# hartikainen/mujoco_mpc

Measured on AMD Instinct MI355X. Metric: candidate rollouts/s (horizon x samples), higher is better.
Workload: dtype f64

## Files before the change

mujoco_mpc_amd/csrc/constraint.h:

```cpp
#pragma once
DEV double impedance(const double *solimp_in, double pos, double margin) {
  double si0 = d_clip(solimp_in[0], 0.0001, 0.9999), si1 = d_clip(solimp_in[1], 0.0001, 0.9999);
  double si2 = fmax(0.0, solimp_in[2]), si3 = d_clip(solimp_in[3], 0.0001, 0.9999), si4 = fmax(1.0, solimp_in[4]);
  if (si0 == si1 || si2 <= D_MINVAL) return 0.5 * (si0 + si1);
  double x = d_div(pos - margin, si2);
  if (x < 0) x = -x;
  if (x >= 1) return si1;
  if (x == 0) return si0;
  double y;
  if (si4 == 1) y = x;
  else {
    int low = x <= si3;
    double m = low ? si3 : 1 - si3, u = low ? x : 1 - x;
    double a = d_div(1.0, d_pow_small(m, si4 - 1));
    double w = a * d_pow_small(u, si4);
    y = low ? w : 1 - w;
  }
  return si0 + y * (si1 - si0);
}

DEV double ball_angle(double *axis, const double *quat) {
  axis[0] = quat[1]; axis[1] = quat[2]; axis[2] = quat[3];
  double s = sqrt(axis[0] * axis[0] + axis[1] * axis[1] + axis[2] * axis[2]);
  if (s < D_MINVAL) { axis[0] = 1; axis[1] = 0; axis[2] = 0; } else { axis[0] /= s; axis[1] /= s; axis[2] /= s; }
// ... 180 lines not shown
        for (int w = MI(tendon_adr)[t2]; w < MI(tendon_adr)[t2] + MI(tendon_num)[t2]; w++) { int qa = MI(wrap_qposadr)[w]; dif += MD(wrap_prm)[w] * (c.qpos[qa] - MDH(qpos0)[qa]); }
        double deriv = ep[1] + dif * (2 * ep[2] + dif * (3 * ep[3] + dif * 4 * ep[4]));
        for (int w = MI(tendon_adr)[t2]; w < MI(tendon_adr)[t2] + MI(tendon_num)[t2]; w++) c.efc_J[r0 * nvp + MI(wrap_dofadr)[w]] -= deriv * MD(wrap_prm)[w];
      }
    } else {
      int b1 = et[1], b2 = et[2];
      const int weld = et[0] == 1;
      double p1[3], p2[3], quat[4], quat1[4];
      d_mulmatvec3(p1, c.xmat + 9 * b1, weld ? ep + 3 : ep); d_mulmatvec3(p2, c.xmat + 9 * b2, weld ? ep : ep + 3);
      for (int q = 0; q < 3; q++) { p1[q] += c.xpos[3 * b1 + q]; p2[q] += c.xpos[3 * b2 + q]; }
      if (weld) {
        d_mulquat(quat, c.xquat + 4 * b1, ep + 6);
        quat1[0] = c.xquat[4 * b2]; for (int q = 1; q < 4; q++) quat1[q] = -c.xquat[4 * b2 + q];
      }
      for (int d = 0; d < nv; d++) {
        unsigned long long bit = 1ull << d;
        int in1 = (MDM()[b1] & bit) != 0, in2 = (MDM()[b2] & bit) != 0;
        if (!in1 && !in2) continue;
        const double *cd = c.cdof + 6 * d;
        double jp[3] = {0, 0, 0}, off[3], t[3];
        if (in1) { d_sub3(off, p1, c.subtree_com + 3 * MIH(body_rootid)[b1]); d_cross(t, cd, off); for (int q = 0; q < 3; q++) jp[q] += cd[3 + q] + t[q]; }
        if (in2) { d_sub3(off, p2, c.subtree_com + 3 * MIH(body_rootid)[b2]); d_cross(t, cd, off); for (int q = 0; q < 3; q++) jp[q] -= cd[3 + q] + t[q]; }
        for (int q = 0; q < 3; q++) c.efc_J[(r0 + q) * nvp + d] = jp[q];
        if (weld) {
          double ax[4] = {0, 0, 0, 0}, tq[4], q3[4];
          if (in1) for (int q = 0; q < 3; q++) ax[1 + q] = cd[q];
          if (in2) for (int q = 0; q < 3; q++) ax[1 + q] -= cd[q];
          d_mulquat(tq, quat1, ax); d_mulquat(q3, tq, quat);
          for (int q = 0; q < 3; q++) c.efc_J[(r0 + 3 + q) * nvp + d] = ep[10] * (0.5 * q3[1 + q]);
        }
      }
    }
  }
  PFOR(rr, ntf_end - neq_end) {
    int r = neq_end + rr, t = MI(tfric_id)[c.efc_id[r]];
    for (int w = MI(tendon_adr)[t]; w < MI(tendon_adr)[t] + MI(tendon_num)[t]; w++) c.efc_J[r * nvp + MI(wrap_dofadr)[w]] = MD(wrap_prm)[w];
  }
  PFOR(rr, nball_end - ntf_end) {
    int r = ntf_end + rr, j = c.efc_id[r], da = MIH(jnt_dofadr)[j];
    double axis[3];
    ball_angle(axis, c.qpos + MIH(jnt_qposadr)[j]);
    for (int k = 0; k < 3; k++) c.efc_J[r * nvp + da + k] = -axis[k];
  }
  PFOR(rr, ntl_end - ntl0) {
    int r = ntl0 + rr, t = c.efc_id[r];
    double sg = c.efc_floss[r];
    for (int w = MI(tendon_adr)[t]; w < MI(tendon_adr)[t] + MI(tendon_num)[t]; w++) c.efc_J[r * nvp + MI(wrap_dofadr)[w]] = sg * MD(wrap_prm)[w];
    c.efc_floss[r] = 0;
  }
  SYNC();
  *nsingle_out = nlim_end; *n_nc_out = ntl_end;
}

DEV void make_contact_rows(Ctx &c, int n_nc) {
  const DevModel &M = *c.M;
  int nv = M.nv, nvp = M.nvp;
  int nefc = n_nc;
  for (int base = 0; base < c.ncon; base += NLANE) {
    int ci = base + LANE, dim = 0;
    if (ci < c.ncon) {
      dim = c.con_i[ci * CONI_STRIDE];
      if (dim > 1 && M.cone != 1) dim = 2 * (dim - 1);
    }
    int tot, off = wave_excl_scan(dim, &tot);
    if (nefc + tot > M.nefcmax) { c.warning |= WARN_CNSTRFULL; c.ncon = base; break; }
    if (ci < c.ncon) {
      int r0 = nefc + off;
      c.con_i[ci * CONI_STRIDE + 3] = r0;
      int g1 = c.con_i[ci * CONI_STRIDE + 1], g2 = c.con_i[ci * CONI_STRIDE + 2];
      int b1 = MI(geom_bodyid)[g1], b2 = MI(geom_bodyid)[g2];
      double tran = MDH(body_invweight0)[2 * b1] + MDH(body_invweight0)[2 * b2];
      double rot = MDH(body_invweight0)[2 * b1 + 1] + MDH(body_invweight0)[2 * b2 + 1];
      const double *cc = c.contact + ci * c.M->con_stride;
      int cdim = c.con_i[ci * CONI_STRIDE];
      int pyr = (cdim > 1 && M.cone != 1);
      for (int k = 0; k < dim; k++) {
        c.efc_type[r0 + k] = cdim == 1 ? CNSTR_CONTACT_FRICTIONLESS : (pyr ? CNSTR_CONTACT_PYRAMIDAL : CNSTR_CONTACT_ELLIPTIC);
        c.efc_id[r0 + k] = EFC_CON_ID(ci, cdim, r0);
        c.efc_floss[r0 + k] = 0; c.efc_pos[r0 + k] = cc[CON_DIST]; c.efc_margin[r0 + k] = cc[CON_INCLUDEMARGIN];
        if (pyr) { double mu = cc[CON_FRICTION + k / 2]; c.efc_diag[r0 + k] = tran + mu * mu * (k < 4 ? tran : rot); }
        else c.efc_diag[r0 + k] = k < 3 ? tran : rot;
      }
    }
    nefc += tot;
  }
  c.nefc = nefc;
  int crossflag = 0;
  PFOR(ci, c.ncon) {
    unsigned long long m1 = MPM()[MI(geom_bodyid)[c.con_i[ci * CONI_STRIDE + 1]]];
    unsigned long long m2 = MPM()[MI(geom_bodyid)[c.con_i[ci * CONI_STRIDE + 2]]];
    unsigned long long u = m1 | m2;
    if (u != m1 && u != m2) crossflag = 1;
  }
  c.cross = wave_or_i(crossflag) | M.limit_cross;
  SYNC();
  PFOR(e, (nefc - n_nc) * nvp) c.efc_J[n_nc * nvp + e] = 0;
  SYNC();
  int je_ci = LANE / nv, je_d = LANE - je_ci * nv;
  const int je_sq = NLANE / nv, je_sr = NLANE - je_sq * nv;
  for (int e = LANE; e < c.ncon * nv; e += NLANE, je_ci += je_sq, je_d += je_sr) {
    if (je_d >= nv) { je_d -= nv; je_ci++; }
    const int ci = je_ci, d = je_d;
    const int *cin = c.con_i + ci * CONI_STRIDE;
    int dim = cin[0], r0 = cin[3];
    int pyr = (dim > 1 && M.cone != 1);
    int b1 = MI(geom_bodyid)[cin[1]], b2 = MI(geom_bodyid)[cin[2]];
    unsigned long long bit = 1ull << d;
    int in1 = (MDM()[b1] & bit) != 0, in2 = (MDM()[b2] & bit) != 0;
    if (!in1 && !in2) continue;
    const double *cc = c.contact + ci * c.M->con_stride;
    const double *cd = c.cdof + 6 * d;
    double jp[3] = {0, 0, 0}, jr[3] = {0, 0, 0};
    if (in2) {
      double off[3], t[3];
      d_sub3(off, cc + CON_POS, c.subtree_com + 3 * MIH(body_rootid)[b2]);
      d_cross(t, cd, off);
      jp[0] += cd[3] + t[0]; jp[1] += cd[4] + t[1]; jp[2] += cd[5] + t[2];
      jr[0] += cd[0]; jr[1] += cd[1]; jr[2] += cd[2];
    }
    if (in1) {
      double off[3], t[3];
      d_sub3(off, cc + CON_POS, c.subtree_com + 3 * MIH(body_rootid)[b1]);
      d_cross(t, cd, off);
      jp[0] -= cd[3] + t[0]; jp[1] -= cd[4] + t[1]; jp[2] -= cd[5] + t[2];
      jr[0] -= cd[0]; jr[1] -= cd[1]; jr[2] -= cd[2];
    }
    if (pyr) {
      double jn = cc[CON_FRAME] * jp[0] + cc[CON_FRAME + 1] * jp[1] + cc[CON_FRAME + 2] * jp[2];
      for (int k = 1; k < dim; k++) {
        const double *ax = cc + CON_FRAME + 3 * (k % 3);
        const double *jj = k < 3 ? jp : jr;
        double jk = ax[0] * jj[0] + ax[1] * jj[1] + ax[2] * jj[2], mu = cc[CON_FRICTION + k - 1];
        c.efc_J[(r0 + 2 * (k - 1)) * nvp + d] = jn + mu * jk;
        c.efc_J[(r0 + 2 * (k - 1) + 1) * nvp + d] = jn - mu * jk;
      }
    } else {
      for (int k = 0; k < dim; k++) {
        const double *ax = cc + CON_FRAME + 3 * (k % 3);
        const double *jj = k < 3 ? jp : jr;
        c.efc_J[(r0 + k) * nvp + d] = ax[0] * jj[0] + ax[1] * jj[1] + ax[2] * jj[2];
      }
    }
  }
  SYNC();
}

DEV void make_impedance(Ctx &c, int r0, int r1, int with_contacts) {
  const DevModel &M = *c.M;
  int nv = M.nv, nvp = M.nvp;
  PFOR(rr, r1 - r0) {
    int r = r0 + rr;
    int type = c.efc_type[r], id = c.efc_id[r];
    double vel = 0;
    if (type == CNSTR_FRICTION_DOF) vel = c.qvel[id];
    else
// ... 78 lines not shown
```

mujoco_mpc_amd/csrc/core.h:

```cpp
#pragma once
#include "dmath.h"
#include "model.h"
#include "linalg.h"
#include "philox.h"

#ifdef MJPC_EMU
static thread_local double *g_emu_lds = nullptr;
static thread_local int g_emu_r = 0;
typedef const KParams *KP;
DEV const KParams *kp_generic(KP k) { return k; }
DEV double *lds_base() { return g_emu_lds; }
DEV int cand_index() { return g_emu_r; }
DEV int uniform_i(int v) { return v; }
#else
extern __shared__ __align__(16) double g_lds[];
typedef const __attribute__((address_space(4))) KParams *KP;
DEV const KParams *kp_generic(KP k) {
  unsigned long long v = (unsigned long long)k;
  unsigned lo = __builtin_amdgcn_readfirstlane((unsigned)v), hi = __builtin_amdgcn_readfirstlane((unsigned)(v >> 32));
  KP u = (KP)(((unsigned long long)hi << 32) | lo);
  return (const KParams *)u;
}
DEV double *lds_base() { return g_lds; }
DEV int cand_index() { return (int)blockIdx.x; }
// ... 233 lines not shown
    for (int k = 0; k < 9; k++) { c.xmat[k] = (k % 4 == 0) ? 1.0 : 0.0; c.ximat[k] = c.xmat[k]; }
    for (int k = 0; k < 6; k++) { c.cvel[k] = 0; c.cfrc[k] = 0; c.cacc[k] = (k >= 3) ? -M.gravity[k - 3] : 0.0; }
    for (int k = 0; k < MISC_INTS; k++) c.misc[k] = 0;
#if defined(MJPC_PROFILE) && !defined(MJPC_EMU)
    for (int q = 0; q < NPROF; q++) c.prof[q] = 0;
    c.prof[NPROF] = (long long)__builtin_amdgcn_s_memtime();
#endif
  }
  c.time = K->time;
  ctx_close(c);
}

template <int NVT>
DEV_NOINLINE void ph_head(KP Kc, int t, int last) {
  Ctx c; ctx_open(c, Kc);
  const KParams *K = c.K;
  const DevModel &M = *c.M;
  Rows R = out_rows(K);
  int nu = M.nu;
  if (!last) {
    PFOR(k, nu) {
      double a = spline_sample(c.knot_times, c.knot_values, K->P, nu, K->interp, c.time, k);
      a = d_clip(a, MD(actuator_ctrlrange)[2 * k], MD(actuator_ctrlrange)[2 * k + 1]);
      c.ctrl[k] = a; R.actions[t * nu + k] = a;
    }
    SYNC();
    if (bad_values(c.qpos, M.nq)) c.warning |= WARN_BADQPOS;
    if (bad_values(c.qvel, M.nv)) c.warning |= WARN_BADQVEL;
    if (c.warning) { if (LANE == 0) c.misc[MISC_BAD_STATE] = 1; ctx_close(c); return; }
    if (K->xfrc_std > 0) {
      double rate = exp(-M.timestep / K->xfrc_rate), scale = K->xfrc_std * sqrt(1 - rate * rate);
      unsigned gi = (unsigned)(K->offset + cand_index());
      int n6 = 6 * M.nbody;
      PFOR(i, n6) c.xfrc[i] = rate * c.xfrc[i] + scale * philox_normal(K->seed, K->stream ^ XFRC_STREAM, gi, (unsigned)(t * n6 + i));
    }
  }
  PROF(c, 0);
  kinematics(c); PROF(c, 1);
#if !MJPC_SIDE_COM
  com_pos(c);
#endif
  PROF(c, 2);
  ctx_close(c);
}
DEV_NOINLINE void ph_constraints(KP Kc, int t) {
  Ctx c; ctx_open(c, Kc);
  collision(c); PROF(c, 4);
  int nsingle, n_nc;
#if MJPC_HELPER
#if MJPC_SIDE_COM
  if (!flag_wait(c.misc + HX_COM, t + 1)) c.warning |= WARN_SYNC;
#endif
  if (!flag_wait(c.misc + HX_NCROWS, t + 1)) c.warning |= WARN_SYNC;
  nsingle = uniform_i(c.misc[HX_NC_NSINGLE]); n_nc = uniform_i(c.misc[HX_NC_ROWS]);
  c.nsingle = nsingle;
  make_contact_rows(c, n_nc); PROF(c, 5);
  make_impedance(c, n_nc, c.nefc, 1); PROF(c, 7);
#else
  make_noncontact_rows(c, &nsingle, &n_nc);
  c.nsingle = nsingle;
  make_contact_rows(c, n_nc); PROF(c, 5);
  make_impedance(c, 0, c.nefc, 1); PROF(c, 7);
#endif
  ctx_close(c);
}
#if MJPC_HELPER
DEV_NOINLINE void ph_noncontact(KP Kc, int t) {
  Ctx c; ctx_open(c, Kc, 1);
  int nsingle, n_nc;
#if MJPC_SIDE_COM
  if (c.M->neq_connect) { if (!flag_wait(c.misc + HX_COM, t + 1)) c.warning |= WARN_SYNC; }
#endif
  make_noncontact_rows(c, &nsingle, &n_nc);
  if (LANE == 0) { c.misc[HX_NC_NSINGLE] = nsingle; c.misc[HX_NC_ROWS] = n_nc; }
  flag_set(c.misc + HX_NCROWS, t + 1);
  PROFW(c, 1);
  make_impedance(c, 0, n_nc, 0);
  PROFW(c, 4);
  if (!flag_wait(c.misc + HX_SWEEP, t + 1)) c.warning |= WARN_SYNC;
  subtree_sums(c, 1);
  flag_set(c.misc + HX_SUBSUM, t + 1);
  PROFW(c, 5);
  ctx_close(c);
}
#endif
template <int NVT>
DEV_NOINLINE void ph_smooth(KP Kc, int t) {
  Ctx c; ctx_open(c, Kc, 1);
#if MJPC_HELPER
#if MJPC_SIDE_COM
  kinematics_rest(c);
  com_pos(c);
  flag_set(c.misc + HX_COM, t + 1);
#endif
  velocity_stage<NVT>(c, Kc, t + 1);
#else
  crb_and_factor<NVT>(c); PROF(c, 3);
  velocity_stage<NVT>(c, Kc, 0); PROF(c, 6);
#endif
  ctx_close(c);
}
#if MJPC_HELPER
template <int NVT>
DEV_NOINLINE void ph_inertia(KP Kc, int t) {
  Ctx c; ctx_open(c, Kc, 1);
#if MJPC_SIDE_COM
  if (!flag_wait(c.misc + HX_COM, t + 1)) c.warning |= WARN_SYNC;
#endif
  crb_and_factor<NVT>(c);
  flag_set(c.misc + HX_MFACT, t + 1);
  ctx_close(c);
}
#endif
template <int NVT>
DEV_NOINLINE void ph_solve(KP Kc, int last, int t) {
  Ctx c; ctx_open(c, Kc);
  c.hseq = t * 256;
  solve_constraints<NVT>(c); PROF(c, 8);
#if MJPC_HELPER
  if (NVT > 0) { if (c.M->cone == 1) flag_set(c.misc + HX_JOBW, JOBW(++c.hseq, 0, 0)); }
  else {
    if (LANE == 0) c.misc[HX_UNREAD_KIND] = 0;
    flag_set(c.misc + HX_UNREAD_SEQ, ++c.hseq);
  }
#endif
  if (!last && !(c.warning & (WARN_CONTACTFULL | WARN_CNSTRFULL)) && bad_values(c.qacc, c.M->nv)) c.warning |= WARN_BADQACC;
  ctx_close(c);
}
template <int NVT>
DEV_NOINLINE void ph_noslip(KP Kc, int last) {
  Ctx c; ctx_open(c, Kc);
  if (!(c.warning & (WARN_CONTACTFULL | WARN_CNSTRFULL | WARN_SYNC | WARN_BADQACC))) {
    noslip_pass<NVT>(c);
    if (!last && bad_values(c.qacc, c.M->nv)) c.warning |= WARN_BADQACC;
  }
  ctx_close(c);
}
#if MJPC_HELPER
template <int NVT>
DEV_NOINLINE void ph_solve_helper(KP Kc, int t) {
  Ctx c; ctx_open(c, Kc, 1);
  int k = WAVE_ID() - 1;
  static_for<0, MJPC_NH>([&](auto Kc_) { constexpr int KK = decltype(Kc_)::value; if (k == KK) solver_helper_loop<NVT, KK>(Kc, c, t * 256); });
}
#endif

struct CostOut { double cost; int warning; };
DEV_NOINLINE CostOut ph_residual_cost(KP Kc, int t, int last) {
  Ctx c; ctx_open(c, Kc, 1);
  const KParams *K = c.K;
  const DevModel &M = *c.M;
  const DevTask &T = M.task;
  Rows R = out_rows(K);
  if (last) PFOR(k, M.nu) R.actions[t * M.nu + k] = (K->H > 1) ? c.ctrl[k] : 0.0;
  if (t == 0 && cand_index() == 0 && K->frame) {
    int nb = M.nbody, ns = M.nsite;
    double *f = K->frame;
    PFOR(i, 3 * nb) { f[i] = c.xpos[i]; f[12 * nb + 3 * ns + i] = c.subtree_com[i]; f[15 * nb + 3 * ns + i] = c.subtree_linvel[i]; }
    PFOR(i, 9 * nb) f[3 * nb + i] = c.xmat[i];
    PFOR(i, 3 * ns) f[12 * nb + i] = c.site_xpos[i];
  }
  task_residual(c, c.residual); PROF(c, 9); PROFW(c, 9);
  PFOR(i, R.nr) R.residual[t * R.nr + i] = c.residual[i];
// ... 349 lines not shown
```

mujoco_mpc_amd/csrc/dynamics.h:

```cpp
#pragma once
DEV void vel_body(Ctx &c, int i) {
  const DevModel &M = *c.M;
  double cvel[6];
  for (int k = 0; k < 6; k++) cvel[k] = c.cvel[6 * MIH(body_parentid)[i] + k];
  int bda = MIH(body_dofadr)[i];
  for (int j = MIH(body_jntadr)[i]; j < MIH(body_jntadr)[i] + MIH(body_jntnum)[i]; j++) {
    int type = MIH(jnt_type)[j];
    if (type == 0) {
      for (int k = 0; k < 18; k++) c.cdof_dot[6 * bda + k] = 0;
      for (int k = 0; k < 3; k++) for (int q = 0; q < 6; q++) cvel[q] += c.cdof[6 * (bda + k) + q] * c.qvel[bda + k];
      bda += 3;
    }
    if (type == 0 || type == 1) {
      for (int k = 0; k < 3; k++) {
        double r[6];
        d_crossmotion(r, cvel, c.cdof + 6 * (bda + k));
        for (int q = 0; q < 6; q++) c.cdof_dot[6 * (bda + k) + q] = r[q];
      }
      for (int k = 0; k < 3; k++) for (int q = 0; q < 6; q++) cvel[q] += c.cdof[6 * (bda + k) + q] * c.qvel[bda + k];
      bda += 3;
    } else {
      double r[6];
      d_crossmotion(r, cvel, c.cdof + 6 * bda);
      for (int q = 0; q < 6; q++) c.cdof_dot[6 * bda + q] = r[q];
// ... 15 lines not shown
  for (int k = 0; k < 6; k++) c.cfrc[6 * i + k] = t1[k] + t3[k];
  double off[3], v[3];
  d_sub3(off, c.xipos + 3 * i, c.subtree_com + 3 * MIH(body_rootid)[i]);
  d_cross(v, cvel, off);
  d_add3(v, v, cvel + 3);
  d_scl3(c.bodytmp + 3 * i, v, MDH(body_mass)[i]);
}

DEV void vel_compose(Ctx &c, int i, double *cvel, double *a, int store) {
  const DevModel &M = *c.M;
  int bda = MIH(body_dofadr)[i];
  for (int j = MIH(body_jntadr)[i]; j < MIH(body_jntadr)[i] + MIH(body_jntnum)[i]; j++) {
    int type = MIH(jnt_type)[j];
    if (type == 0) {
      if (store) for (int k = 0; k < 18; k++) c.cdof_dot[6 * bda + k] = 0;
      for (int k = 0; k < 3; k++) for (int q = 0; q < 6; q++) a[q] += 0.0 * c.qvel[bda + k];
      for (int k = 0; k < 3; k++) for (int q = 0; q < 6; q++) cvel[q] += c.cdof[6 * (bda + k) + q] * c.qvel[bda + k];
      bda += 3;
    }
    if (type == 0 || type == 1) {
      for (int k = 0; k < 3; k++) {
        double r[6];
        d_crossmotion(r, cvel, c.cdof + 6 * (bda + k));
        if (store) for (int q = 0; q < 6; q++) c.cdof_dot[6 * (bda + k) + q] = r[q];
        for (int q = 0; q < 6; q++) a[q] += r[q] * c.qvel[bda + k];
      }
      for (int k = 0; k < 3; k++) for (int q = 0; q < 6; q++) cvel[q] += c.cdof[6 * (bda + k) + q] * c.qvel[bda + k];
      bda += 3;
    } else {
      double r[6];
      d_crossmotion(r, cvel, c.cdof + 6 * bda);
      if (store) for (int q = 0; q < 6; q++) c.cdof_dot[6 * bda + q] = r[q];
      for (int q = 0; q < 6; q++) a[q] += r[q] * c.qvel[bda];
      for (int q = 0; q < 6; q++) cvel[q] += c.cdof[6 * bda + q] * c.qvel[bda];
      bda++;
    }
  }
  if (!store) return;
  for (int k = 0; k < 6; k++) { c.cvel[6 * i + k] = cvel[k]; c.cacc[6 * i + k] = a[k]; }
  double t1[6], t2[6], t3[6];
  d_mulinertvec(t1, c.cinert + 10 * i, a);
  d_mulinertvec(t2, c.cinert + 10 * i, cvel);
  d_crossforce(t3, cvel, t2);
  for (int k = 0; k < 6; k++) c.cfrc[6 * i + k] = t1[k] + t3[k];
  double off[3], v[3];
  d_sub3(off, c.xipos + 3 * i, c.subtree_com + 3 * MIH(body_rootid)[i]);
  d_cross(v, cvel, off);
  d_add3(v, v, cvel + 3);
  d_scl3(c.bodytmp + 3 * i, v, MDH(body_mass)[i]);
}

DEV void subtree_sums(Ctx &c, int part) {
  const DevModel &M = *c.M;
  int per = part ? 6 : 3;
  PFOR(e, M.nbody * per) {
    int b = e / per, k = e - per * b;
    if (k < 3) {
      int kc = k + 3 * part;
      double s = 0;
      if (b > 0) for (int q = MIH(subtree_adr)[b]; q < MIH(subtree_adr)[b + 1]; q++) s += c.cfrc[6 * MIH(subtree_list)[q] + kc];
      c.cfrc_sub[6 * b + kc] = s;
    } else {
      int kk = k - 3;
      double s = 0;
      for (int q = MIH(subtree_adr)[b] + (b == 0); q < MIH(subtree_adr)[b + 1]; q++) s += c.bodytmp[3 * MIH(subtree_list)[q] + kk];
      c.subtree_linvel[3 * b + kk] = s / fmax(D_MINVAL, MDH(body_subtreemass)[b]);
    }
  }
}

DEV double rs_moment(Ctx &c, const int *ri, const double *w, int d) {
  const DevModel &M = *c.M;
  const int s = ri[1], r = ri[2], bs = ri[3], br = ri[4];
  const unsigned long long common = (unsigned long long)(unsigned)ri[5] | ((unsigned long long)(unsigned)ri[6] << 32);
  const int in_s = (int)((MDM()[bs] >> d) & 1ull), in_r = (int)((MDM()[br] >> d) & 1ull);
  if ((!in_s && !in_r) || ((common >> d) & 1ull)) return 0.0;
  const double *cd = c.cdof + 6 * d;
  double jp[3] = {0, 0, 0}, off[3], t[3];
  if (in_s) { d_sub3(off, c.site_xpos + 3 * s, c.subtree_com + 3 * MIH(body_rootid)[bs]); d_cross(t, cd, off); for (int q = 0; q < 3; q++) jp[q] += cd[3 + q] + t[q]; }
  if (in_r) { d_sub3(off, c.site_xpos + 3 * r, c.subtree_com + 3 * MIH(body_rootid)[br]); d_cross(t, cd, off); for (int q = 0; q < 3; q++) jp[q] -= cd[3 + q] + t[q]; }
  return jp[0] * w[0] + jp[1] * w[1] + jp[2] * w[2];
}
DEV double actuator_force_of(Ctx &c, int i, double u) {
  double force = MD(actuator_gainprm)[3 * i] * u;
  if (MI(actuator_biastype)[i] == 1) {
    double length = 0, velocity = 0;
    for (int e = MI(act_adr)[i]; e < MI(act_adr)[i + 1]; e++) {
      double cf = MD(act_coef)[e];
      length += cf * c.qpos[MI(act_qpos)[e]]; velocity += cf * c.qvel[MI(act_dof)[e]];
    }
    if (c.M->nrsact > 0 && MI(rsact_of)[i] >= 0) {
      const int k = MI(rsact_of)[i];
      const int *ri = MI(rsact_i) + 7 * k;
      double w[3], vec[3];
      d_mulmatvec3(w, c.xmat + 9 * ri[4], MD(rsact_g) + 3 * k);
      d_sub3(vec, c.site_xpos + 3 * ri[1], c.site_xpos + 3 * ri[2]);
      length = w[0] * vec[0] + w[1] * vec[1] + w[2] * vec[2];
      for (int d = 0; d < c.M->nv; d++) velocity += rs_moment(c, ri, w, d) * c.qvel[d];
    }
    force += MD(actuator_biasprm)[3 * i] + MD(actuator_biasprm)[3 * i + 1] * length + MD(actuator_biasprm)[3 * i + 2] * velocity;
  }
  if (MI(actuator_forcelimited)[i]) force = d_clip(force, MD(actuator_forcerange)[2 * i], MD(actuator_forcerange)[2 * i + 1]);
  return force;
}

DEV_NOINLINE void ph_smooth_extras(KP Kc) {
  Ctx c; ctx_open(c, Kc, 1);
  const DevModel &M = *c.M;
  const int nv = M.nv;
  if (M.nactfrc > 0) {
    PFOR(k, M.nactfrc) {
      int dd = MI(actfrc_dof)[k];
      double act = 0;
      for (int q = MI(dact_adr)[dd]; q < MI(dact_adr)[dd + 1]; q++) { int e = MI(dact_e)[q]; act += MD(act_coef)[e] * c.actuator_force[MI(act_of)[e]]; }
      c.qfrc_smooth[dd] += d_clip(act, MD(actfrc_range)[2 * k], MD(actfrc_range)[2 * k + 1]) - act;
    }
    SYNC();
  }
  if (M.fluid) {
    PFOR(b, M.nbody) {
// ... 62 lines not shown
    PFOR(d, nv) {
      double acc = c.qfrc_smooth[d];
      const double *cd = c.cdof + 6 * d;
      for (int k = 0; k < M.nsiteact; k++) {
        int a = MI(sact_i)[3 * k], s = MI(sact_i)[3 * k + 1], b = MI(sact_i)[3 * k + 2];
        if (!((MDM()[b] >> d) & 1ull)) continue;
        double f[3], tq[3], off[3], t[3];
        d_mulmatvec3(f, c.xmat + 9 * b, MD(sact_g) + 6 * k); d_mulmatvec3(tq, c.xmat + 9 * b, MD(sact_g) + 6 * k + 3);
        d_sub3(off, c.site_xpos + 3 * s, c.subtree_com + 3 * MIH(body_rootid)[b]);
        d_cross(t, cd, off);
        acc += c.actuator_force[a] * ((cd[3] + t[0]) * f[0] + (cd[4] + t[1]) * f[1] + (cd[5] + t[2]) * f[2] + cd[0] * tq[0] + cd[1] * tq[1] + cd[2] * tq[2]);
      }
      c.qfrc_smooth[d] = acc;
    }
    SYNC();
  }
  if (M.nrsact > 0) {
    PFOR(d, nv) {
      double acc = c.qfrc_smooth[d];
      for (int k = 0; k < M.nrsact; k++) {
        const int *ri = MI(rsact_i) + 7 * k;
        double w[3];
        d_mulmatvec3(w, c.xmat + 9 * ri[4], MD(rsact_g) + 3 * k);
        acc += rs_moment(c, ri, w, d) * c.actuator_force[ri[0]];
      }
      c.qfrc_smooth[d] = acc;
    }
    SYNC();
  }
  if (M.ntendon_passive > 0) {
    PFOR(d, nv) {
      double acc = c.qfrc_smooth[d];
      for (int e = 0; e < M.ntendon_passive; e++) {
        int t = MI(tpass_id)[e];
        double coef = 0, length = 0, velocity = 0;
        for (int w = MI(tendon_adr)[t]; w < MI(tendon_adr)[t] + MI(tendon_num)[t]; w++) {
          double cf = MD(wrap_prm)[w];
          length += cf * c.qpos[MI(wrap_qposadr)[w]]; velocity += cf * c.qvel[MI(wrap_dofadr)[w]];
          if (MI(wrap_dofadr)[w] == d) coef += cf;
        }
        if (coef == 0) continue;
        const double *pr = MD(tpass_prm) + 4 * e;
        double frc = 0;
        if (length > pr[3]) frc = pr[0] * (pr[3] - length); else if (length < pr[2]) frc = pr[0] * (pr[2] - length);
        frc -= pr[1] * velocity;
        acc += coef * frc;
      }
      c.qfrc_smooth[d] = acc;
    }
    SYNC();
  }
}

template <int NVT>
DEV void velocity_stage(Ctx &c, KP Kc, int mfact_seq) {
  const DevModel &M = *c.M;
  int nv = M.nv;
#ifdef MJPC_LEAN_LDS
  if (LANE < 6) { c.cfrc[LANE] = 0; c.cacc[LANE] = (LANE >= 3) ? -M.gravity[LANE - 3] : 0.0; }
  SYNC();
#endif
  if constexpr (NVT == 27 || NVT == 33) {
    PFOR(b, M.nbody) {
      if (b == 0) continue;
      double cvel[6], acc[6];
      for (int k = 0; k < 6; k++) { cvel[k] = c.cvel[k]; acc[k] = c.cacc[k]; }
      for (int q = MIH(chain_adr)[b]; q < MIH(chain_adr)[b + 1]; q++) {
        int a = MIH(chain_list)[q];
        vel_compose(c, a, cvel, acc, a == b);
      }
    }
    SYNC();
  } else {
    for (int l = 0; l < M.nlevel; l++) {
      int a = MIH(level_adr)[l], n = MIH(level_adr)[l + 1] - a;
      PFOR(k, n) vel_body(c, MIH(level_body)[a + k]);
      SYNC();
    }
  }
  PROFW(c, 1);
#if MJPC_HELPER
  flag_set(c.misc + HX_SWEEP, mfact_seq);
  subtree_sums(c, 0);
#else
  subtree_sums(c, 0); subtree_sums(c, 1);
#endif
  PROFW(c, 4);
  PFOR(i, M.nu) {
    double ctrl = c.ctrl[i];
    if (MI(actuator_ctrllimited)[i]) ctrl = d_clip(ctrl, MD(actuator_ctrlrange)[2 * i], MD(actuator_ctrlrange)[2 * i + 1]);
    c.actuator_force[i] = actuator_force_of(c, i, ctrl);
  }
  if (M.na) {
    PFOR(i, M.nu) {
      int dt = MI(actuator_dyntype)[i];
      if (dt) {
        double ctrl = c.ctrl[i];
        if (MI(actuator_ctrllimited)[i]) ctrl = d_clip(ctrl, MD(actuator_ctrlrange)[2 * i], MD(actuator_ctrlrange)[2 * i + 1]);
        int a = MI(actuator_actadr)[i];
        double act = C_ACT(c)[a];
        C_ACTDOT(c)[a] = dt == DYN_INTEGRATOR ? ctrl : d_div(ctrl - act, fmax(D_MINVAL, MD(actuator_dynprm)[i]));
        c.actuator_force[i] = actuator_force_of(c, i, act);
      }
    }
  }
#if MJPC_HELPER
  if (!flag_wait(c.misc + HX_SUBSUM, mfact_seq)) c.warning |= WARN_SYNC;
#endif
  SYNC();
  PFOR(d, nv) {
    const double *cd = c.cdof + 6 * d, *cf = c.cfrc_sub + 6 * MIH(dof_bodyid)[d];
    double bias = cd[0]*cf[0] + cd[1]*cf[1] + cd[2]*cf[2] + cd[3]*cf[3] + cd[4]*cf[4] + cd[5]*cf[5];
    c.qfrc_bias[d] = bias;
    double act = 0;
    for (int q = MI(dact_adr)[d]; q < MI(dact_adr)[d + 1]; q++) { int e = MI(dact_e)[q]; act += MD(act_coef)[e] * c.actuator_force[MI(act_of)[e]]; }
    c.qfrc_smooth[d] = act - bias - MD(dof_damping)[d] * c.qvel[d];
  }
  SYNC();
  PFOR(j, M.njnt) {
    double k = MDH(jnt_stiffness)[j];
    int type = MIH(jnt_type)[j];
    if (k != 0 && (type == 2 || type == 3)) {
      int qa = MIH(jnt_qposadr)[j];
      c.qfrc_smooth[MIH(jnt_dofadr)[j]] -= k * (c.qpos[qa] - MDH(qpos_spring)[qa]);
    }
  }
  SYNC();
  if (M.smooth_extras) ph_smooth_extras(Kc);
  if (c.K->xfrc_std > 0) {
    PFOR(d, nv) {
      const double *cd = c.cdof + 6 * d;
      int bd = MIH(dof_bodyid)[d];
      double acc = c.qfrc_smooth[d];
      for (int q = MIH(subtree_adr)[bd]; q < MIH(subtree_adr)[bd + 1]; q++) {
        int b = MIH(subtree_list)[q];
        const double *f = c.xfrc + 6 * b;
        double off[3], tt[3];
        d_sub3(off, c.xipos + 3 * b, c.subtree_com + 3 * MIH(body_rootid)[b]);
        d_cross(tt, cd, off);
        acc += (cd[3] + tt[0]) * f[0] + (cd[4] + tt[1]) * f[1] + (cd[5] + tt[2]) * f[2] + cd[0] * f[3] + cd[1] * f[4] + cd[2] * f[5];
      }
      c.qfrc_smooth[d] = acc;
    }
    SYNC();
  }
  PFOR(d, nv) c.qacc_smooth[d] = c.qfrc_smooth[d];
  PROFW(c, 5);
  if (mfact_seq && !flag_wait(c.misc + HX_MFACT, mfact_seq)) c.warning |= WARN_SYNC;
  PROFW(c, 7);
  chol_solve<NVT>(c.qL, c.Linv, c.qacc_smooth, nv, M.nvp, M.tree_ok);
  PROFW(c, 8);
}

#include "solver.h"
```

mujoco_mpc_amd/csrc/kinematics.h:

```cpp
#pragma once
DEV void kin_joint_local(Ctx &c, int j, double *jq) {
  const DevModel &M = *c.M;
  int type = MIH(jnt_type)[j], qa = MIH(jnt_qposadr)[j];
  if (type == 3) {
    double ax[3];
    d_copy3(ax, MDH(jnt_axis) + 3 * j);
    d_axisangle2quat(jq + 4 * j, ax, c.qpos[qa] - MDH(qpos0)[qa]);
  } else if (type == 1) {
    d_normalize4(c.qpos + qa);
    d_copy4(jq + 4 * j, c.qpos + qa);
  } else if (type == 0) {
    d_normalize4(c.qpos + qa + 3);
  }
}
DEV void kin_compose(Ctx &c, int i, const double *jq, const double *ppos, const double *pquat, const double *pmat, int have_parent,
                     double *xpos, double *xquat, double *xm, int store) {
  const DevModel &M = *c.M;
  int jntnum = MIH(body_jntnum)[i], jntadr = MIH(body_jntadr)[i];
  int mid = MIH(body_mocapid)[i];
  if (mid >= 0) {
    d_copy3(xpos, c.mocap_pos + 3 * mid);
    d_copy4(xquat, c.mocap_quat + 4 * mid);
    d_normalize4(xquat);
  } else if (jntnum == 1 && MIH(jnt_type)[jntadr] == 0) {
// ... 2 lines not shown
    d_copy4(xquat, c.qpos + qa + 3);
    if (store) {
      d_copy3(c.xanchor + 3 * jntadr, xpos);
      d_copy3(c.xaxis + 3 * jntadr, MDH(jnt_axis) + 3 * jntadr);
    }
  } else {
    if (have_parent) {
      d_mulmatvec3(xpos, pmat, MDH(body_pos) + 3 * i);
      d_add3(xpos, xpos, ppos);
      d_mulquat(xquat, pquat, MDH(body_quat) + 4 * i);
    } else {
      d_copy3(xpos, MDH(body_pos) + 3 * i);
      d_copy4(xquat, MDH(body_quat) + 4 * i);
    }
    if (jntnum > 0) {
      double m[9];
      d_quat2mat(m, xquat);
      for (int j = jntadr; j < jntadr + jntnum; j++) {
        int qa = MIH(jnt_qposadr)[j], type = MIH(jnt_type)[j];
        double vec[3], ax[3], jp[3], xax[3], xan[3];
        d_copy3(ax, MDH(jnt_axis) + 3 * j); d_copy3(jp, MDH(jnt_pos) + 3 * j);
        d_mulmatvec3(xax, m, ax);
        d_mulmatvec3(vec, m, jp);
        d_add3(xan, vec, xpos);
        if (store) { d_copy3(c.xaxis + 3 * j, xax); d_copy3(c.xanchor + 3 * j, xan); }
        if (type == 2) {
          d_addtoscl3(xpos, xax, c.qpos[qa] - MDH(qpos0)[qa]);
        } else {
          double qloc[4], t[4];
          d_copy4(qloc, jq + 4 * j);
          d_mulquat(t, xquat, qloc);
          d_copy4(xquat, t);
          d_quat2mat(m, xquat);
          d_mulmatvec3(vec, m, jp);
          d_sub3(xpos, xan, vec);
        }
      }
    }
  }
  d_normalize4(xquat);
  d_quat2mat(xm, xquat);
  if (store) {
    d_copy3(c.xpos + 3 * i, xpos);
    d_copy4(c.xquat + 4 * i, xquat);
    for (int k = 0; k < 9; k++) c.xmat[9 * i + k] = xm[k];
  }
}

#if MJPC_HELPER && !defined(MJPC_LEAN_LDS)
#define MJPC_SIDE_COM 1
#else
#define MJPC_SIDE_COM 0
#endif
DEV void kin_frames_sites(Ctx &c) {
  const DevModel &M = *c.M;
  PFOR(i, M.nbody) {
    if (i == 0) continue;
    double v[3], q[4], ip[3], iq[4], xm[9];
    d_copy3(ip, MDH(body_ipos) + 3 * i); d_copy4(iq, MDH(body_iquat) + 4 * i);
    d_mulmatvec3(v, c.xmat + 9 * i, ip);
    d_add3(c.xipos + 3 * i, v, c.xpos + 3 * i);
    d_mulquat(q, c.xquat + 4 * i, iq);
    d_quat2mat(xm, q);
    for (int k = 0; k < 9; k++) c.ximat[9 * i + k] = xm[k];
  }
  PFOR(s, M.nsite) {
    int b = MI(site_bodyid)[s];
    double v[3], sp[3];
    d_copy3(sp, MD(site_pos) + 3 * s);
    d_mulmatvec3(v, c.xmat + 9 * b, sp);
    d_add3(c.site_xpos + 3 * s, v, c.xpos + 3 * b);
  }
}
DEV void kinematics_rest(Ctx &c) { kin_frames_sites(c); SYNC(); }

DEV void kinematics(Ctx &c) {
  const DevModel &M = *c.M;
  double *jq = c.cdof_dot;
  PFOR(j, M.njnt) kin_joint_local(c, j, jq);
  SYNC();
  PFOR(b, M.nbody) {
    if (b == 0) continue;
    double ppos[3], pquat[4], pmat[9], xpos[3], xquat[4], xm[9];
    int have = 0;
    for (int q = MIH(chain_adr)[b]; q < MIH(chain_adr)[b + 1]; q++) {
      int a = MIH(chain_list)[q];
      kin_compose(c, a, jq, ppos, pquat, pmat, have, xpos, xquat, xm, a == b);
      d_copy3(ppos, xpos); d_copy4(pquat, xquat);
      for (int k = 0; k < 9; k++) pmat[k] = xm[k];
      have = 1;
    }
  }
  SYNC();
#if !MJPC_SIDE_COM
  kin_frames_sites(c);
#endif
  PFOR(g, M.ngeom) {
    int b = MI(geom_bodyid)[g];
    double v[3], q[4], gp[3], gq[4], xm[9];
    d_copy3(gp, MD(geom_pos) + 3 * g); d_copy4(gq, MD(geom_quat) + 4 * g);
    d_mulmatvec3(v, c.xmat + 9 * b, gp);
    d_add3(c.geom_xpos + 3 * g, v, c.xpos + 3 * b);
    d_mulquat(q, c.xquat + 4 * b, gq);
    d_quat2mat(xm, q);
    for (int k = 0; k < 9; k++) c.geom_xmat[9 * g + k] = xm[k];
  }
  SYNC();
}
DEV void com_pos(Ctx &c) {
  const DevModel &M = *c.M;
  PFOR(b, M.nbody) {
    double s[3] = {0, 0, 0};
    for (int k = MIH(subtree_adr)[b]; k < MIH(subtree_adr)[b + 1]; k++) {
      int cb = MIH(subtree_list)[k];
      d_addtoscl3(s, c.xipos + 3 * cb, MDH(body_mass)[cb]);
    }
    double sm = MDH(body_subtreemass)[b];
    if (sm < D_MINVAL) d_copy3(c.subtree_com + 3 * b, c.xipos + 3 * b);
    else d_scl3(c.subtree_com + 3 * b, s, 1.0 / sm);
  }
  SYNC();
  PFOR(b, M.nbody) {
    if (b == 0) { for (int k = 0; k < 10; k++) c.cinert[k] = 0; continue; }
    double off[3], ine[3], r[10];
    d_sub3(off, c.xipos + 3 * b, c.subtree_com + 3 * MIH(body_rootid)[b]);
    d_copy3(ine, MDH(body_inertia) + 3 * b);
    d_inertcom(r, ine, c.ximat + 9 * b, off, MDH(body_mass)[b]);
    for (int k = 0; k < 10; k++) c.cinert[10 * b + k] = r[k];
  }
  PFOR(j, M.njnt) {
    int b = MIH(jnt_bodyid)[j], da = MIH(jnt_dofadr)[j], type = MIH(jnt_type)[j];
    double off[3];
    d_sub3(off, c.subtree_com + 3 * MIH(body_rootid)[b], c.xanchor + 3 * j);
    int skip = 0;
    if (type == 0) {
      for (int k = 0; k < 18; k++) c.cdof[6 * da + k] = 0;
      for (int k = 0; k < 3; k++) c.cdof[6 * (da + k) + 3 + k] = 1;
      skip = 3;
    }
    if (type == 0 || type == 1) {
      const double *xm = c.xmat + 9 * b;
      for (int k = 0; k < 3; k++) {
        double ax[3] = {xm[k], xm[k + 3], xm[k + 6]}, cr[3];
        double *cd = c.cdof + 6 * (da + k + skip);
        d_cross(cr, ax, off);
        d_copy3(cd, ax); d_copy3(cd + 3, cr);
      }
    } else if (type == 2) {
// ... 41 lines not shown
```

mujoco_mpc_amd/csrc/model.h:

```cpp
#pragma once
#include <stdint.h>

#define CON_STRIDE_ELLIPTIC 45
#define NVP_OF(n) ((((n) + 1)) | 1)
#define CON_STRIDE_PLAIN 27
#define CON_DIST 0
#define CON_POS 1
#define CON_FRAME 4
#define CON_INCLUDEMARGIN 13
#define CON_FRICTION 14
#define CON_SOLREF 19
#define CON_SOLIMP 21
#define CON_MU 26
#define CON_H 27
#define CONI_STRIDE 4
#define MAX_ACTIVE_PAIRS 192
#define EFC_CON_ID(ci, dim, r0) ((ci) | ((dim) << 8) | ((r0) << 16))
#define EFC_CON_CI(id) ((id) & 255)
#define EFC_CON_DIM(id) (((id) >> 8) & 255)
#define EFC_CON_R0(id) ((id) >> 16)

template <int N> struct DofTree { static constexpr bool known = false; static constexpr int parent(int) { return -1; } static constexpr int real_parent(int) { return -1; } };
template <> struct DofTree<18> {
  static constexpr bool known = true;
// ... 101 lines not shown
  const int *tfric_id;
  const double *tfric_prm;
  const double *key_qpos, *key_mpos;
  const int *geom_dataid, *mesh_vertadr, *mesh_vertnum;
  const double *mesh_vert;
  const int *hfield_nrow, *hfield_ncol, *hfield_adr;
  const double *hfield_size, *hfield_data;
  const int *level_adr, *level_body;
  const int *subtree_adr, *subtree_list;
  const int *chain_adr, *chain_list;
  const int *mpair_i, *mpair_j;
  const int *hpair_i, *hpair_j;
  const int *zpair_i, *zpair_j;
  const unsigned long long *body_dofmask;
  const unsigned long long *body_patmask;
  const int *pair_gg; const double *pair_bp;
  const int *fric_dof, *limit_jnt, *limit_ball, *ray_geom;
  DevTask task;
};

#define LAY_SLAB(off) (-1 - (off))
#define SPILL_NOSLIP 1u
#define SPILL_EFC_JA 2u
#define SPILL_EFC_J 4u
#define SPILL_CONTACT 8u
#define SPILL_EFC_VEC 16u
#define SPILL_EVERY 31u
enum { SPILL_NONE = 0, SPILL_AUTO = 1, SPILL_ALL = 2 };
#define MISC_INTS 48
enum {
  MISC_NCON = 0,
  MISC_NEFC = 1,
  MISC_NSINGLE = 2,
  MISC_WARNING = 3,
  MISC_SOLVER_ITER = 4,
  MISC_SUM_ITER = 5,
  MISC_MAX_NCON = 6,
  MISC_MAX_NEFC = 7,
  MISC_CROSS = 8,
  MISC_QH_DENSE = 9,
  MISC_BAD_STATE = 10,
  MISC_WARN_OTHERS = 11,
  HX_UNREAD_SEQ = 12,
  HX_UNREAD_KIND = 13,
  HX_LSREC = 17,
  HX_JOBW = 18,
  HX_SUBSUM = 19,
  HX_MFACT = 22,
  HX_CSM = 23,
  HX_NCROWS = 24,
  HX_NC_NSINGLE = 25,
  HX_NC_ROWS = 26,
  HX_SWEEP = 27,
  HX_WDONE = 36,
  HX_WDONE_END = 38,
  HX_COM = 44,
  HX_NITEMS = 45,
  HX_HEAVY = 46
};
static_assert(HX_HEAVY < MISC_INTS && HX_WDONE_END <= MISC_INTS, "misc[] slot beyond MISC_INTS");
struct Lay {
  int qpos, qvel, ctrl, qacc, qacc_ws, qacc_smooth, qfrc_smooth, qfrc_bias, qfrc_constraint, actuator_force;
  int mocap_pos, mocap_quat;
  int xpos, xquat, xmat, xipos, ximat, xanchor, xaxis, geom_xpos, geom_xmat, site_xpos;
  int subtree_com, cinert, crb, cdof, cvel, cdof_dot, cacc, cfrc, cfrc_sub, subtree_linvel, bodytmp;
  int qM, qL, qH, Linv, Hinv;
  int efc_J, efc_JA, efc_D, efc_R, efc_aref, efc_force, efc_jar, efc_jv, efc_floss, efc_pos, efc_margin, efc_diag;
  int contact;
  int Ma, grad, Mgrad, search, Mv, vtmp, sgl;
  int knot_times, knot_values, residual, terms, red, prof, scr_a, scr_b;
  int xfrc;
  int noslip;
  int mc_d, mc_i;
  int ints;
  int i_efc_type, i_efc_id, i_efc_state, i_efc_dof, i_con, i_active, i_misc, i_hpair;
  int total_doubles;
};

struct KParams {
  DevModel M;
  Lay L;
  const int *ibase; const double *dbase;
  int cache_i, cache_d;
  const double *state, *mocap, *knot_times, *knot_values, *noise_eps, *noise_std, *cand_knots;
  const double *userdata; int nuserdata;
  double xfrc_std, xfrc_rate;
  const int *noise_sel;
  double time, sigma0, sigma1;
  unsigned long long seed, stream;
  int P, interp, H, N, offset, nlocal, use_device_noise, nominal_index;
  double *ckpt; int ckpt_stride, tier;
  int retry;
  int fault;
  double *states, *actions, *times, *residual, *costs, *trace, *knots, *returns;
  int *failure, *diag;
  double *frame;
  long long *prof;
  double *slab; long long slab_stride;
};
```

Baseline: 28900.

## Split contact row construction across helper waves and move actuator forces off critical path

Breaks make_contact_rows into scan, headers, cross-flag and Jacobian pieces. With helper waves enabled, the noncontact helper builds the contact row headers and the factor helper computes the second half of the contact Jacobian, with new flag slots coordinating them. Actuator forces (and sites, when no actuator needs them) move to the noncontact helper, and subtree_sums is rebalanced into even halves. The aim is to shorten the main wave's critical path, at the cost of extra flag waits and cross-wave synchronization that could stall if the helpers are busy.

```diff
diff --git a/mujoco_mpc_amd/csrc/constraint.h b/mujoco_mpc_amd/csrc/constraint.h
--- a/mujoco_mpc_amd/csrc/constraint.h
+++ b/mujoco_mpc_amd/csrc/constraint.h
@@ -256,9 +256,8 @@
   *nsingle_out = nlim_end; *n_nc_out = ntl_end;
 }
 
-DEV void make_contact_rows(Ctx &c, int n_nc) {
-  const DevModel &M = *c.M;
-  int nv = M.nv, nvp = M.nvp;
+DEV void contact_row_scan(Ctx &c, int n_nc) {
+  const DevModel &M = *c.M;
   int nefc = n_nc;
   for (int base = 0; base < c.ncon; base += NLANE) {
     int ci = base + LANE, dim = 0;
@@ -268,27 +267,35 @@
     }
     int tot, off = wave_excl_scan(dim, &tot);
     if (nefc + tot > M.nefcmax) { c.warning |= WARN_CNSTRFULL; c.ncon = base; break; }
-    if (ci < c.ncon) {
-      int r0 = nefc + off;
-      c.con_i[ci * CONI_STRIDE + 3] = r0;
-      int g1 = c.con_i[ci * CONI_STRIDE + 1], g2 = c.con_i[ci * CONI_STRIDE + 2];
-      int b1 = MI(geom_bodyid)[g1], b2 = MI(geom_bodyid)[g2];
-      double tran = MDH(body_invweight0)[2 * b1] + MDH(body_invweight0)[2 * b2];
-      double rot = MDH(body_invweight0)[2 * b1 + 1] + MDH(body_invweight0)[2 * b2 + 1];
-      const double *cc = c.contact + ci * c.M->con_stride;
-      int cdim = c.con_i[ci * CONI_STRIDE];
-      int pyr = (cdim > 1 && M.cone != 1);
-      for (int k = 0; k < dim; k++) {
-        c.efc_type[r0 + k] = cdim == 1 ? CNSTR_CONTACT_FRICTIONLESS : (pyr ? CNSTR_CONTACT_PYRAMIDAL : CNSTR_CONTACT_ELLIPTIC);
-        c.efc_id[r0 + k] = EFC_CON_ID(ci, cdim, r0);
-        c.efc_floss[r0 + k] = 0; c.efc_pos[r0 + k] = cc[CON_DIST]; c.efc_margin[r0 + k] = cc[CON_INCLUDEMARGIN];
-        if (pyr) { double mu = cc[CON_FRICTION + k / 2]; c.efc_diag[r0 + k] = tran + mu * mu * (k < 4 ? tran : rot); }
-        else c.efc_diag[r0 + k] = k < 3 ? tran : rot;
-      }
-    }
+    if (ci < c.ncon) c.con_i[ci * CONI_STRIDE + 3] = nefc + off;
     nefc += tot;
   }
   c.nefc = nefc;
+}
+DEV void contact_row_headers(Ctx &c, int ncon) {
+  const DevModel &M = *c.M;
+  PFOR(ci, ncon) {
+    int r0 = c.con_i[ci * CONI_STRIDE + 3];
+    int g1 = c.con_i[ci * CONI_STRIDE + 1], g2 = c.con_i[ci * CONI_STRIDE + 2];
+    int b1 = MI(geom_bodyid)[g1], b2 = MI(geom_bodyid)[g2];
+    double tran = MDH(body_invweight0)[2 * b1] + MDH(body_invweight0)[2 * b2];
+    double rot = MDH(body_invweight0)[2 * b1 + 1] + MDH(body_invweight0)[2 * b2 + 1];
+    const double *cc = c.contact + ci * c.M->con_stride;
+    int cdim = c.con_i[ci * CONI_STRIDE];
+    int pyr = (cdim > 1 && M.cone != 1);
+    int dim = pyr ? 2 * (cdim - 1) : cdim;
+    for (int k = 0; k < dim; k++) {
+      c.efc_type[r0 + k] = cdim == 1 ? CNSTR_CONTACT_FRICTIONLESS : (pyr ? CNSTR_CONTACT_PYRAMIDAL : CNSTR_CONTACT_ELLIPTIC);
+      c.efc_id[r0 + k] = EFC_CON_ID(ci, cdim, r0);
+      c.efc_floss[r0 + k] = 0; c.efc_pos[r0 + k] = cc[CON_DIST]; c.efc_margin[r0 + k] = cc[CON_INCLUDEMARGIN];
+      if (pyr) { double mu = cc[CON_FRICTION + k / 2]; c.efc_diag[r0 + k] = tran + mu * mu * (k < 4 ? tran : rot); }
+      else c.efc_diag[r0 + k] = k < 3 ? tran : rot;
+    }
+  }
+  SYNC();
+}
+DEV void contact_cross_flag(Ctx &c) {
+  const DevModel &M = *c.M;
   int crossflag = 0;
   PFOR(ci, c.ncon) {
     unsigned long long m1 = MPM()[MI(geom_bodyid)[c.con_i[ci * CONI_STRIDE + 1]]];
@@ -298,13 +305,19 @@
   }
   c.cross = wave_or_i(crossflag) | M.limit_cross;
   SYNC();
-  PFOR(e, (nefc - n_nc) * nvp) c.efc_J[n_nc * nvp + e] = 0;
+}
+DEV void contact_jacobian(Ctx &c, int ci0, int ci1, int ncon, int nefc) {
+  const DevModel &M = *c.M;
+  int nv = M.nv, nvp = M.nvp;
+  const int rbeg = ci0 < ncon ? uniform_i(c.con_i[ci0 * CONI_STRIDE + 3]) : nefc;
+  const int rend = ci1 < ncon ? uniform_i(c.con_i[ci1 * CONI_STRIDE + 3]) : nefc;
+  PFOR(e, (rend - rbeg) * nvp) c.efc_J[rbeg * nvp + e] = 0;
   SYNC();
   int je_ci = LANE / nv, je_d = LANE - je_ci * nv;
   const int je_sq = NLANE / nv, je_sr = NLANE - je_sq * nv;
-  for (int e = LANE; e < c.ncon * nv; e += NLANE, je_ci += je_sq, je_d += je_sr) {
+  for (int e = LANE; e < (ci1 - ci0) * nv; e += NLANE, je_ci += je_sq, je_d += je_sr) {
     if (je_d >= nv) { je_d -= nv; je_ci++; }
-    const int ci = je_ci, d = je_d;
+    const int ci = ci0 + je_ci, d = je_d;
     const int *cin = c.con_i + ci * CONI_STRIDE;
     int dim = cin[0], r0 = cin[3];
     int pyr = (dim > 1 && M.cone != 1);
diff --git a/mujoco_mpc_amd/csrc/core.h b/mujoco_mpc_amd/csrc/core.h
--- a/mujoco_mpc_amd/csrc/core.h
+++ b/mujoco_mpc_amd/csrc/core.h
@@ -309,14 +309,26 @@
   if (!flag_wait(c.misc + HX_COM, t + 1)) c.warning |= WARN_SYNC;
 #endif
   if (!flag_wait(c.misc + HX_NCROWS, t + 1)) c.warning |= WARN_SYNC;
+  PROF(c, 10);
   nsingle = uniform_i(c.misc[HX_NC_NSINGLE]); n_nc = uniform_i(c.misc[HX_NC_ROWS]);
   c.nsingle = nsingle;
-  make_contact_rows(c, n_nc); PROF(c, 5);
+  contact_row_scan(c, n_nc);
+  if (LANE == 0) { c.misc[HX_CR_NCON] = c.ncon; c.misc[HX_CR_NEFC] = c.nefc; }
+  flag_set(c.misc + HX_CROWS, t + 1);
+  contact_cross_flag(c); PROF(c, 18);
+  contact_jacobian(c, 0, c.ncon / 2, c.ncon, c.nefc);
+  if (!flag_wait(c.misc + HX_CJAC, t + 1)) c.warning |= WARN_SYNC;
+  if (!flag_wait(c.misc + HX_CHDR, t + 1)) c.warning |= WARN_SYNC;
+  PROF(c, 5);
   make_impedance(c, n_nc, c.nefc, 1); PROF(c, 7);
 #else
   make_noncontact_rows(c, &nsingle, &n_nc);
   c.nsingle = nsingle;
-  make_contact_rows(c, n_nc); PROF(c, 5);
+  contact_row_scan(c, n_nc);
+  contact_row_headers(c, c.ncon);
+  contact_cross_flag(c);
+  contact_jacobian(c, 0, c.ncon, c.ncon, c.nefc);
+  PROF(c, 5);
   make_impedance(c, 0, c.nefc, 1); PROF(c, 7);
 #endif
   ctx_close(c);
@@ -328,13 +340,26 @@
 #if MJPC_SIDE_COM
   if (c.M->neq_connect) { if (!flag_wait(c.misc + HX_COM, t + 1)) c.warning |= WARN_SYNC; }
 #endif
+  if (c.M->nrsact == 0) {
+#if MJPC_SIDE_COM
+    kin_sites(c);
+#endif
+    actuator_forces(c);
+  }
+  PROFW(c, 8);
   make_noncontact_rows(c, &nsingle, &n_nc);
   if (LANE == 0) { c.misc[HX_NC_NSINGLE] = nsingle; c.misc[HX_NC_ROWS] = n_nc; }
   flag_set(c.misc + HX_NCROWS, t + 1);
   PROFW(c, 1);
   make_impedance(c, 0, n_nc, 0);
   PROFW(c, 4);
+  if (!flag_wait(c.misc + HX_CROWS, t + 1)) c.warning |= WARN_SYNC;
+  PROFW(c, 9);
+  contact_row_headers(c, uniform_i(c.misc[HX_CR_NCON]));
+  flag_set(c.misc + HX_CHDR, t + 1);
+  PROFW(c, 10);
   if (!flag_wait(c.misc + HX_SWEEP, t + 1)) c.warning |= WARN_SYNC;
+  PROFW(c, 7);
   subtree_sums(c, 1);
   flag_set(c.misc + HX_SUBSUM, t + 1);
   PROFW(c, 5);
@@ -349,6 +374,7 @@
   kinematics_rest(c);
   com_pos(c);
   flag_set(c.misc + HX_COM, t + 1);
+  PROFW(c, 17);
 #endif
   velocity_stage<NVT>(c, Kc, t + 1);
 #else
@@ -363,9 +389,18 @@
   Ctx c; ctx_open(c, Kc, 1);
 #if MJPC_SIDE_COM
   if (!flag_wait(c.misc + HX_COM, t + 1)) c.warning |= WARN_SYNC;
+  PROFW(c, 7);
 #endif
   crb_and_factor<NVT>(c);
   flag_set(c.misc + HX_MFACT, t + 1);
+  if (!flag_wait(c.misc + HX_CROWS, t + 1)) c.warning |= WARN_SYNC;
+  PROFW(c, 8);
+  {
+    const int ncon = uniform_i(c.misc[HX_CR_NCON]), nefc = uniform_i(c.misc[HX_CR_NEFC]);
+    contact_jacobian(c, ncon / 2, ncon, ncon, nefc);
+  }
+  flag_set(c.misc + HX_CJAC, t + 1);
+  PROFW(c, 9);
   ctx_close(c);
 }
 #endif
diff --git a/mujoco_mpc_amd/csrc/dynamics.h b/mujoco_mpc_amd/csrc/dynamics.h
--- a/mujoco_mpc_amd/csrc/dynamics.h
+++ b/mujoco_mpc_amd/csrc/dynamics.h
@@ -91,20 +91,17 @@
 
 DEV void subtree_sums(Ctx &c, int part) {
   const DevModel &M = *c.M;
-  int per = part ? 6 : 3;
-  PFOR(e, M.nbody * per) {
-    int b = e / per, k = e - per * b;
-    if (k < 3) {
-      int kc = k + 3 * part;
-      double s = 0;
-      if (b > 0) for (int q = MIH(subtree_adr)[b]; q < MIH(subtree_adr)[b + 1]; q++) s += c.cfrc[6 * MIH(subtree_list)[q] + kc];
-      c.cfrc_sub[6 * b + kc] = s;
-    } else {
-      int kk = k - 3;
-      double s = 0;
-      for (int q = MIH(subtree_adr)[b] + (b == 0); q < MIH(subtree_adr)[b + 1]; q++) s += c.bodytmp[3 * MIH(subtree_list)[q] + kk];
-      c.subtree_linvel[3 * b + kk] = s / fmax(D_MINVAL, MDH(body_subtreemass)[b]);
-    }
+  const int n = 9 * M.nbody, half = (n + 1) >> 1;
+  const int e1 = part ? n : half;
+  for (int e = (part ? half : 0) + LANE; e < e1; e += NLANE) {
+    const int b = e / 9, k = e - 9 * b, mom = k >= 6;
+    const double *src = mom ? c.bodytmp + (k - 6) : c.cfrc + k;
+    const int stride = mom ? 3 : 6;
+    const int q0 = MIH(subtree_adr)[b] + (b == 0), q1 = (b == 0 && !mom) ? q0 : MIH(subtree_adr)[b + 1];
+    double s = 0;
+    for (int q = q0; q < q1; q++) s += src[stride * MIH(subtree_list)[q]];
+    if (mom) c.subtree_linvel[3 * b + k - 6] = s / fmax(D_MINVAL, MDH(body_subtreemass)[b]);
+    else c.cfrc_sub[6 * b + k] = s;
   }
 }
 
@@ -273,6 +270,28 @@
   }
 }
 
+DEV void actuator_forces(Ctx &c) {
+  const DevModel &M = *c.M;
+  PFOR(i, M.nu) {
+    double ctrl = c.ctrl[i];
+    if (MI(actuator_ctrllimited)[i]) ctrl = d_clip(ctrl, MD(actuator_ctrlrange)[2 * i], MD(actuator_ctrlrange)[2 * i + 1]);
+    c.actuator_force[i] = actuator_force_of(c, i, ctrl);
+  }
+  if (M.na) {
+    PFOR(i, M.nu) {
+      int dt = MI(actuator_dyntype)[i];
+      if (dt) {
+        double ctrl = c.ctrl[i];
+        if (MI(actuator_ctrllimited)[i]) ctrl = d_clip(ctrl, MD(actuator_ctrlrange)[2 * i], MD(actuator_ctrlrange)[2 * i + 1]);
+        int a = MI(actuator_actadr)[i];
+        double act = C_ACT(c)[a];
+        C_ACTDOT(c)[a] = dt == DYN_INTEGRATOR ? ctrl : d_div(ctrl - act, fmax(D_MINVAL, MD(actuator_dynprm)[i]));
+        c.actuator_force[i] = actuator_force_of(c, i, act);
+      }
+    }
+  }
+}
+
 template <int NVT>
 DEV void velocity_stage(Ctx &c, KP Kc, int mfact_seq) {
   const DevModel &M = *c.M;
@@ -307,28 +326,16 @@
   subtree_sums(c, 0); subtree_sums(c, 1);
 #endif
   PROFW(c, 4);
-  PFOR(i, M.nu) {
-    double ctrl = c.ctrl[i];
-    if (MI(actuator_ctrllimited)[i]) ctrl = d_clip(ctrl, MD(actuator_ctrlrange)[2 * i], MD(actuator_ctrlrange)[2 * i + 1]);
-    c.actuator_force[i] = actuator_force_of(c, i, ctrl);
-  }
-  if (M.na) {
-    PFOR(i, M.nu) {
-      int dt = MI(actuator_dyntype)[i];
-      if (dt) {
-        double ctrl = c.ctrl[i];
-        if (MI(actuator_ctrllimited)[i]) ctrl = d_clip(ctrl, MD(actuator_ctrlrange)[2 * i], MD(actuator_ctrlrange)[2 * i + 1]);
-        int a = MI(actuator_actadr)[i];
-        double act = C_ACT(c)[a];
-        C_ACTDOT(c)[a] = dt == DYN_INTEGRATOR ? ctrl : d_div(ctrl - act, fmax(D_MINVAL, MD(actuator_dynprm)[i]));
-        c.actuator_force[i] = actuator_force_of(c, i, act);
-      }
-    }
-  }
+#if MJPC_HELPER
+  if (M.nrsact > 0)
+#endif
+  actuator_forces(c);
+  PROFW(c, 18);
 #if MJPC_HELPER
   if (!flag_wait(c.misc + HX_SUBSUM, mfact_seq)) c.warning |= WARN_SYNC;
 #endif
   SYNC();
+  PROFW(c, 19);
   PFOR(d, nv) {
     const double *cd = c.cdof + 6 * d, *cf = c.cfrc_sub + 6 * MIH(dof_bodyid)[d];
     double bias = cd[0]*cf[0] + cd[1]*cf[1] + cd[2]*cf[2] + cd[3]*cf[3] + cd[4]*cf[4] + cd[5]*cf[5];
diff --git a/mujoco_mpc_amd/csrc/kinematics.h b/mujoco_mpc_amd/csrc/kinematics.h
--- a/mujoco_mpc_amd/csrc/kinematics.h
+++ b/mujoco_mpc_amd/csrc/kinematics.h
@@ -78,7 +78,7 @@
 #else
 #define MJPC_SIDE_COM 0
 #endif
-DEV void kin_frames_sites(Ctx &c) {
+DEV void kin_frames(Ctx &c) {
   const DevModel &M = *c.M;
   PFOR(i, M.nbody) {
     if (i == 0) continue;
@@ -90,6 +90,9 @@
     d_quat2mat(xm, q);
     for (int k = 0; k < 9; k++) c.ximat[9 * i + k] = xm[k];
   }
+}
+DEV void kin_sites(Ctx &c) {
+  const DevModel &M = *c.M;
   PFOR(s, M.nsite) {
     int b = MI(site_bodyid)[s];
     double v[3], sp[3];
@@ -98,7 +101,7 @@
     d_add3(c.site_xpos + 3 * s, v, c.xpos + 3 * b);
   }
 }
-DEV void kinematics_rest(Ctx &c) { kin_frames_sites(c); SYNC(); }
+DEV void kinematics_rest(Ctx &c) { kin_frames(c); if (c.M->nrsact > 0) kin_sites(c); SYNC(); }
 
 DEV void kinematics(Ctx &c) {
   const DevModel &M = *c.M;
@@ -119,7 +122,7 @@
   }
   SYNC();
 #if !MJPC_SIDE_COM
-  kin_frames_sites(c);
+  kin_frames(c); kin_sites(c);
 #endif
   PFOR(g, M.ngeom) {
     int b = MI(geom_bodyid)[g];
diff --git a/mujoco_mpc_amd/csrc/model.h b/mujoco_mpc_amd/csrc/model.h
--- a/mujoco_mpc_amd/csrc/model.h
+++ b/mujoco_mpc_amd/csrc/model.h
@@ -177,6 +177,11 @@
   HX_NC_NSINGLE = 25,
   HX_NC_ROWS = 26,
   HX_SWEEP = 27,
+  HX_CROWS = 28,
+  HX_CR_NCON = 29,
+  HX_CR_NEFC = 30,
+  HX_CJAC = 31,
+  HX_CHDR = 32,
   HX_WDONE = 36,
   HX_WDONE_END = 38,
   HX_COM = 44,
```

New measurement: 29290, median of 6. +1.4%, better.
